# frobelbest/BANet

Hardware: AMD Instinct MI355X
Metric: LM iterations/sec (2-frame 640x480 5-level dense BA, 128-coeff depth basis, batch 32) (higher is better)
Workload: dtype f32 (SYRK: fp32 operands as bf16x3 / scaled fp16x2 pieces, fp32 accumulate, <= 2e-7 per entry; roofline.syrk_form)

## Files before the change

### banet_amd/_capi.py

```python
import ctypes
import os

import torch

_HERE = os.path.dirname(os.path.abspath(__file__))
LIB_PATH = os.environ.get("BANET_HIP_LIB") or os.path.join(_HERE, "lib", "libbanet_hip.so")

LEGACY_LM, LEGACY_FIXED, BUNDLE_CAMERA, BUNDLE = 0, 1, 2, 3

_FP = ctypes.c_void_p


class BanetError(RuntimeError):
    pass


class Level(ctypes.Structure):
    _fields_ = [("B", ctypes.c_int32), ("N", ctypes.c_int32), ("C", ctypes.c_int32), ("K", ctypes.c_int32),
                ("H", ctypes.c_int32), ("W", ctypes.c_int32), ("variant", ctypes.c_int32),
                ("dense", ctypes.c_int32), ("tgt_has_grad", ctypes.c_int32), ("normalize_rays", ctypes.c_int32),
                ("scale", ctypes.c_float), ("pairs", ctypes.c_int32), ("flags", ctypes.c_int32), ("policy", ctypes.c_int32),
                ("src", _FP), ("tgt", _FP), ("depth", _FP), ("basis", _FP), ("rays", _FP),
                ("fx", _FP), ("fy", _FP), ("ox", _FP), ("oy", _FP), ("intr", _FP)]

# ... 42 lines not shown
class Mlp(ctypes.Structure):
    _fields_ = [("w", _FP * 5), ("b", _FP * 5)]


class State(ctypes.Structure):
    _fields_ = [("R", _FP), ("T", _FP), ("Wc", _FP), ("iters", _FP), ("ratio", _FP), ("lambda_out", _FP),
                ("delta", _FP)]


class LmParams(ctypes.Structure):
    _fields_ = [("angle_change", ctypes.c_float), ("translation_change", ctypes.c_float),
                ("residual_ratio", ctypes.c_float), ("solver", ctypes.c_int32)]


SOLVER_QR, SOLVER_INVERSE = 0, 1

EXPORTS = {
    "banet_version": (ctypes.c_int, []),
    "banet_error_string": (ctypes.c_char_p, [ctypes.c_int]),
    "banet_equation_construction_workspace_bytes": (ctypes.c_size_t, [ctypes.c_int] * 4),
    "banet_equation_construction_f32": (ctypes.c_int, [_FP] * 5 + [ctypes.c_int] * 4 + [_FP, ctypes.c_size_t, _FP]),
    "banet_equation_construction_grad_workspace_bytes": (ctypes.c_size_t, [ctypes.c_int] * 4),
    "banet_equation_construction_grad_f32": (ctypes.c_int, [_FP] * 8 + [ctypes.c_int] * 4 + [_FP, ctypes.c_size_t, _FP]),
    "banet_resample_f32": (ctypes.c_int, [_FP] * 3 + [ctypes.c_int] * 6 + [_FP]),
    "banet_target_map_f32": (ctypes.c_int, [_FP] * 2 + [ctypes.c_int] * 4 + [_FP]),
    "banet_depth_output_f32": (ctypes.c_int, [_FP] * 4 + [ctypes.c_int] * 3 + [_FP]),
    "banet_resample_grad_workspace_bytes": (ctypes.c_size_t, [ctypes.c_int] * 6),
    "banet_resample_grad_f32": (ctypes.c_int, [_FP] * 5 + [ctypes.c_int] * 7 + [_FP, ctypes.c_size_t, _FP]),
    "banet_depth_output_grad_workspace_bytes": (ctypes.c_size_t, [ctypes.c_int] * 3),
    "banet_depth_output_grad_f32": (ctypes.c_int, [_FP] * 6 + [ctypes.c_int] * 4 + [_FP, ctypes.c_size_t, _FP]),
# ... 18 lines not shown
    "banet_sample_stats_grad_workspace_bytes": (ctypes.c_size_t, [ctypes.c_int] * 5),
    "banet_sample_stats_grad_det_f32": (ctypes.c_int, [_FP] * 4 + [ctypes.c_int] * 5 + [_FP] * 5 + [_FP, ctypes.c_size_t, _FP]),
    "banet_spd_solve_f32": (ctypes.c_int, [_FP] * 3 + [ctypes.c_int] * 2 + [_FP]),
    "banet_dense_adjoint_workspace_bytes": (ctypes.c_size_t, [ctypes.POINTER(Level)]),
    "banet_dense_adjoint_workspace_bytes_ex": (ctypes.c_size_t, [ctypes.POINTER(Level), ctypes.c_int]),
    "banet_dense_adjoint_f32": (ctypes.c_int, [ctypes.POINTER(Level)] + [_FP] * 11 + [_FP, ctypes.c_size_t, _FP]),
    "banet_dense_adjoint_ex_f32": (ctypes.c_int, [ctypes.POINTER(Level)] + [_FP] * 11 + [ctypes.c_int, _FP, ctypes.c_size_t, _FP]),
    "banet_small_step_adjoint_workspace_bytes": (ctypes.c_size_t, [ctypes.c_int] * 6),
    "banet_small_step_adjoint_f32": (ctypes.c_int, [ctypes.c_int] * 6 + [ctypes.c_float, ctypes.POINTER(Mlp)] + [_FP] * 14 +
                                     [ctypes.POINTER(Mlp), _FP, ctypes.c_size_t, _FP]),
    "banet_target_map_adjoint_f32": (ctypes.c_int, [_FP] * 2 + [ctypes.c_int] * 4 + [_FP]),
    "banet_target_map_adjoint_ex_f32": (ctypes.c_int, [_FP] * 2 + [ctypes.c_int] * 5 + [_FP]),
    "banet_build_id": (ctypes.c_char_p, []),
    "banet_gather_selection": (ctypes.c_int, [_FP]),
    "banet_syrk_selection": (ctypes.c_int, [_FP]),
    "banet_profile_ranges": (ctypes.c_int, [ctypes.c_int]),
    "banet_profile_begin": (ctypes.c_int, [ctypes.c_int]),
    "banet_profile_end": (ctypes.c_int, [ctypes.c_int, ctypes.POINTER(ctypes.c_int32), ctypes.POINTER(ctypes.c_int32),
                                         ctypes.POINTER(ctypes.c_double), ctypes.POINTER(ctypes.c_int32)]),
}

_lib = None


def lib():
    global _lib
    if _lib is None:
        if not os.path.exists(LIB_PATH):
            raise BanetError("%s not found: build it with banet_amd/csrc/build.sh (or __graft_entry__.build())"
                             % LIB_PATH)
# ... 40 lines not shown
```

### banet_amd/csrc/api.hip

```cpp
#include "kernels.hpp"

namespace banet {

static bool aligned256(const void* p) { return (reinterpret_cast<uintptr_t>(p) & 255u) == 0; }

static int check_level(const banet_level_t* lv) {
  if (!lv || !lv->src || !lv->tgt || !lv->depth) return BANET_ERR_INVALID_ARG;
  if (lv->variant < BANET_LEGACY_LM || lv->variant > BANET_BUNDLE) return BANET_ERR_INVALID_ARG;
  if (lv->K > 0 && !lv->basis) return BANET_ERR_INVALID_ARG;
  if ((lv->variant == BANET_BUNDLE) != (lv->K > 0)) return BANET_ERR_INVALID_ARG;
  if (lv->pairs < 0 || (lv->policy != BANET_POLICY_THROUGHPUT && lv->policy != BANET_POLICY_BATCH_INVARIANT)) return BANET_ERR_INVALID_ARG;
  if (lv->pairs > 1 && lv->variant != BANET_BUNDLE && lv->variant != BANET_BUNDLE_CAMERA) return BANET_ERR_INVALID_ARG;
  if (lv->dense) {
    if (!lv->intr || !(lv->scale > 0.f)) return BANET_ERR_INVALID_ARG;
  } else {
    if (!lv->rays || !lv->fx || !lv->fy || !lv->ox || !lv->oy) return BANET_ERR_INVALID_ARG;
  }
  return BANET_OK;
}

struct LevelWs {
  float* partials;
  float* AtA;
  float* Atb;
// ... 34 lines not shown
  a.C = lv->C;
  a.K = lv->K;
  a.pairs = npairs(lv);
  a.P = 6 * a.pairs + lv->K;
  a.variant = lv->variant;
  a.l2_base = l2_base;
  a.max_iters = 0;
  a.use_mlp = lv->variant != BANET_LEGACY_FIXED;
  if (mlp) a.mlp = *mlp;
  else
    for (int i = 0; i < 5; ++i) a.mlp.w[i] = a.mlp.b[i] = nullptr;
  a.AtA = AtA;
  a.Atb = Atb;
  a.absres = absres;
  a.nvalid = nvalid;
  a.st = *st;
  a.ctl = nullptr;
  a.queue = nullptr;
  a.nqueue = 0;
  a.bigA = nullptr;
  a.mlp_y = nullptr;
  a.flags = lv->flags;
  banet_lm_params_default(&a.lm);
  return a;
}

static int check_state(const banet_level_t* lv, const banet_mlp_t* mlp, const banet_state_t* st) {
  if (!st || !st->R || !st->T || !st->iters || !st->ratio || !st->lambda_out || !st->delta) return BANET_ERR_INVALID_ARG;
  if (lv->K > 0 && !st->Wc) return BANET_ERR_INVALID_ARG;
  if (lv->variant != BANET_LEGACY_FIXED) {
// ... 126 lines not shown

size_t banet_lm_level_workspace_bytes(const banet_level_t* lv) {
  AsmPlan pl;
  if (plan_assemble(lv, num_cus(), &pl) != BANET_OK) return 0;
  return carve_level(lv, pl, nullptr).total;
}

void banet_lm_params_default(banet_lm_params_t* p) {
  if (!p) return;
  p->angle_change = (float)(0.002 * (3.14 / 180.0));
  p->translation_change = 0.0002f;
  p->residual_ratio = 1.0f;
  p->solver = BANET_SOLVER_QR;
}

constexpr int kRoleSmallLevel = 19200;

int banet_lm_level_f32(const banet_level_t* lv, const banet_mlp_t* mlp, float l2_base, int max_iters,
                       int early_termination, banet_state_t* st, void* ws, size_t ws_bytes, banet_stream_t stream) {
  return banet_lm_level_ex_f32(lv, mlp, l2_base, max_iters, early_termination, nullptr, st, ws, ws_bytes, stream);
}

int banet_lm_level_ex_f32(const banet_level_t* lv, const banet_mlp_t* mlp, float l2_base, int max_iters,
                          int early_termination, const banet_lm_params_t* params, banet_state_t* st, void* ws,
                          size_t ws_bytes, banet_stream_t stream) {
  int rc = check_level(lv);
  if (rc != BANET_OK) return rc;
  rc = check_state(lv, mlp, st);
  if (rc != BANET_OK) return rc;
  if (max_iters < 0) return BANET_ERR_INVALID_ARG;
  AsmPlan pl;
// ... 20 lines not shown
    for (int it = 0; it <= max_iters; ++it) {
      rc = launch_assemble(lv, pl, st->R, st->T, st->Wc, &w.ctl->active, stride, w.partials, w.AtA, w.Atb, w.absres,
                           w.nvalid, s);
      if (rc != BANET_OK) return rc;
      {
        RangeScope r("solve", lv->N);
        rc = launch_solve(a, s);
      }
      if (rc != BANET_OK) return rc;
    }
  } else {
    launch_zero_iters(st->iters, lv->B, s);
    a.queue = assemble_queue(pl, w.partials);
    a.nqueue = 8 * npairs(lv);
    if (a.queue) launch_zero_iters(a.queue, lv->B * a.nqueue, s);
    const int Bsel = selection_batch(lv);
    const bool role = lv->variant == BANET_BUNDLE && mlp != nullptr && a.use_mlp && syrk_runs_mlp_role(pl.s) && lv->C <= 256 &&
                      (lv->C & 3) == 0 && ((long long)Bsel * (pl.s.Gs + 1) <= num_cus() || (Bsel <= 8 && pl.s.Gs >= 16) ||
                       (lv->N <= kRoleSmallLevel && pl.s.Gs >= 4)) &&
                      !(lv->flags & kDevMlpInSolve);
    if (role) {
      a.mlp_y = w.mlp_y;
      if ((long long)Bsel * (pl.s.Gs + 1) > num_cus()) pl.s.Gs -= 1;
    }
    for (int it = 0; it < max_iters; ++it) {
      rc = launch_assemble(lv, pl, st->R, st->T, st->Wc, nullptr, 0, w.partials, w.AtA, w.Atb, w.absres, w.nvalid, s,
                           a.queue == nullptr, role ? mlp : nullptr, role ? w.mlp_y : nullptr, nullptr,
                           pl.s.f16 ? (it == 0 ? (max_iters > 1 ? 2 : 0) : 1) : -1);
      if (rc != BANET_OK) return rc;
      {
        RangeScope r("solve", lv->N);
        rc = launch_solve(a, s);
      }
      if (rc != BANET_OK) return rc;
    }
  }
  return BANET_OK;
}

int banet_resample_f32(const float* data, const float* warp, float* out, int B, int N, int C, int H, int W, int mode,
                       banet_stream_t stream) {
  if (!data || !warp || !out) return BANET_ERR_INVALID_ARG;
  return launch_resample(data, warp, out, B, N, C, H, W, mode, static_cast<hipStream_t>(stream));
// ... 158 lines not shown
int banet_gather_selection(const banet_level_t* lv) {
  GatherPlan pl;
  const int rc = plan_gather(lv, num_cus(), &pl);
  if (rc != BANET_OK) return rc;
  return pl.quad ? 4 : pl.strip ? 3 : pl.patch ? 2 : pl.c128 ? 1 : 0;
}

int banet_syrk_selection(const banet_level_t* lv) {
  AsmPlan pl;
  const int rc = plan_assemble(lv, num_cus(), &pl);
  if (rc != BANET_OK) return rc;
  if (lv->K == 0) return -1000;
  return pl.s.f16 ? 4 : pl.s.direct;
}

int banet_profile_begin(int max_launches) { return profile_begin(max_launches); }

int banet_profile_end(int max_tags, int32_t* tag_points, int32_t* tag_launches, double* tag_ms, int32_t* ntags) {
  return profile_end(max_tags, tag_points, tag_launches, tag_ms, ntags);
}

}
```

### banet_amd/csrc/assemble.hip

```cpp
#include <atomic>
#include <dlfcn.h>

#include <cstdio>
#include <cstdlib>
#include <vector>

#include "kernels.hpp"

namespace banet {

namespace {
struct Profiler {
  bool on = false;
  std::vector<hipEvent_t> ev;
  std::vector<int> tag;
  int used = 0;
} g_prof;

struct Timed {
  hipStream_t s;
  int slot;
  Timed(hipStream_t st, int tag) : s(st), slot(-1) {
    if (g_prof.on && (size_t)(2 * g_prof.used + 1) < g_prof.ev.size()) {
      slot = g_prof.used++;
// ... 105 lines not shown
      (void)hipGetLastError();
      n = kDefault;
    }
    cached[dev].store(n, std::memory_order_relaxed);
  }
  return n;
}

int* assemble_queue(const AsmPlan& pl, void* ws) {
  return pl.g.c128 ? reinterpret_cast<int*>(static_cast<char*>(ws) + pl.g.off_queue) : nullptr;
}

int launch_assemble(const banet_level_t* lv, const AsmPlan& pl, const float* R, const float* T, const float* Wc,
                    const int32_t* active, int active_stride, void* ws, float* AtA, float* Atb, float* absres,
                    float* nvalid, hipStream_t s, bool reset_queue, const banet_mlp_t* role_mlp, float* role_y,
                    unsigned char* mask_out, int f16_stats) {
  char* base = static_cast<char*>(ws);
  float* gpart = reinterpret_cast<float*>(base);
  float* rec = lv->K > 0 ? reinterpret_cast<float*>(base + pl.off_rec) : nullptr;
  float* spart = lv->K > 0 ? reinterpret_cast<float*>(base + pl.off_spart) : nullptr;
  int rc;
  if (reset_queue) prepare_gather(lv, pl.g, gpart, s);
  {
    RangeScope r("gather", lv->N);
    Timed t(s, lv->N);
    rc = launch_gather(lv, pl.g, R, T, Wc, active, active_stride, rec, gpart, s, mask_out);
  }
  if (rc != BANET_OK) return rc;
  const float* gred;
  {
    RangeScope r("fold", lv->N);
// ... 5 lines not shown
    MlpRole mr{};
    if (role_mlp != nullptr && role_y != nullptr && syrk_runs_mlp_role(pl.s)) {
      mr.gpart = gred;
      mr.grows = pl.g.frows;
      mr.gstride = pl.g.pstride;
      mr.mlp = *role_mlp;
      mr.C = lv->C;
      mr.pairs = npairs(lv);
      mr.Nf = (float)lv->N * (float)npairs(lv);
      mr.y = role_y;
    }
    rc = launch_syrk(lv->basis, rec, lv->B, lv->N, lv->K, npairs(lv), pl.s, active, active_stride, spart, s,
                     mr.y != nullptr ? &mr : nullptr, f16_stats);
    if (rc != BANET_OK) return rc;
  }
  RangeScope r("reduce", lv->N);
  launch_reduce2(gred, pl.g.frows, pl.g.pstride, spart, pl.s.Gs, pl.s.pstride, active, active_stride, lv->B, lv->K, lv->C,
                 npairs(lv), AtA, Atb, absres, nvalid, s);
  return hipGetLastError() == hipSuccess ? BANET_OK : BANET_ERR_LAUNCH;
}

}
```

### banet_amd/csrc/kernels.hpp

```cpp
#pragma once
#include "common.hpp"

namespace banet {

constexpr int kUStrideS = 8;

int num_cus();

void prepare_gather(const banet_level_t* lv, const GatherPlan& pl, float* partials, hipStream_t s);
int launch_gather(const banet_level_t* lv, const GatherPlan& pl, const float* R, const float* T, const float* Wc,
                  const int32_t* active, int active_stride, float* rec, float* partials, hipStream_t s,
                  unsigned char* mask_out = nullptr);
const float* finish_gather(const banet_level_t* lv, const GatherPlan& pl, const int32_t* active, int active_stride,
                           float* partials, hipStream_t s);

struct MlpRole {
  const float* gpart;
  int grows, gstride;
  banet_mlp_t mlp;
  int C, pairs;
  float Nf;
  float* y;
};
int launch_syrk_wide(const float* basis, const float* rec, int B, int N, int K, int pairs, int Gs, int pstride,
                     const int32_t* active, int active_stride, float* partials, float* aux, hipStream_t s,
                     const float* colmax = nullptr, const float* recmax = nullptr);
int launch_syrk(const float* basis, const float* rec, int B, int N, int K, int pairs, const SyrkPlan& pl,
                const int32_t* active, int active_stride, float* partials, hipStream_t s, const MlpRole* mr = nullptr,
                int f16_stats = -1);
inline bool syrk_runs_mlp_role(const SyrkPlan& pl) { return pl.direct == 2; }
void launch_reduce2(const float* gpart, int Gg, int gstride, const float* spart, int Gs, int sstride,
                    const int32_t* active, int active_stride, int B, int K, int C, int pairs, float* AtA, float* Atb,
                    float* absres, float* nvalid, hipStream_t s);

int launch_assemble(const banet_level_t* lv, const AsmPlan& pl, const float* R, const float* T, const float* Wc,
                    const int32_t* active, int active_stride, void* ws, float* AtA, float* Atb, float* absres,
                    float* nvalid, hipStream_t s, bool reset_queue = true, const banet_mlp_t* role_mlp = nullptr,
                    float* role_y = nullptr, unsigned char* mask_out = nullptr, int f16_stats = -1);
int* assemble_queue(const AsmPlan& pl, void* ws);
int profile_ranges(int enable);
struct RangeScope {
  bool on;
  RangeScope(const char* role, int n = -1);
  ~RangeScope();
};
int profile_begin(int max_launches);
int profile_end(int max_tags, int32_t* tag_points, int32_t* tag_launches, double* tag_ms, int32_t* ntags);

int launch_resample(const float* data, const float* warp, float* out, int B, int N, int C, int H, int W, int mode,
                    hipStream_t s);
int launch_target_map(const float* img, float* out, int B, int H, int W, int C, hipStream_t s);
int launch_depth_output(const float* init, const float* basis, const float* Wc, float* out, int B, int N, int K,
                        hipStream_t s);
// ... 34 lines not shown
  float Tprev[3];
  int32_t pad_[3];
};
static_assert(sizeof(LmCtl) == 80, "LmCtl layout");

struct SolveArgs {
  int B, N, C, K, P, variant, pairs;
  float l2_base;
  int max_iters;
  banet_mlp_t mlp;
  int use_mlp;
  const float* AtA;
  const float* Atb;
  const float* absres;
  const float* nvalid;
  banet_state_t st;
  LmCtl* ctl;
  float* bigA;
  int* queue;
  int nqueue;
  const float* mlp_y;
  banet_lm_params_t lm;
  int flags;
};
int launch_solve(const SolveArgs& a, hipStream_t s);
int launch_spd_solve(const float* A, const float* rhs, float* x, int B, int P, hipStream_t s);
bool spd_solve_fits(int P);
size_t solve_big_bytes(int B, int P, int C);
void launch_ctl_init(LmCtl* ctl, int32_t* iters, int B, hipStream_t s);
void launch_zero_iters(int32_t* iters, int B, hipStream_t s);
// ... 27 lines not shown
```

### banet_amd/csrc/plan.hpp

```cpp
#pragma once
#include <stddef.h>
#include <stdint.h>

#include <algorithm>

#include "../../include/banet_hip.h"
#include "dev_flags.hpp"

#ifndef BANET_GATHER_WAVES
#define BANET_GATHER_WAVES 3
#endif
#ifndef BANET_G128P_WAVES
#define BANET_G128P_WAVES 2
#endif
#ifndef BANET_G128_WAVES
#define BANET_G128_WAVES 3
#endif

namespace banet {

constexpr int kWave = 64;
constexpr int kTilePix = 64;
constexpr int kBlock = 256;
constexpr int kNumWaves = kBlock / kWave;
// ... 225 lines not shown
};

inline int plan_assemble(const banet_level_t* lv, int cus, AsmPlan* pl) {
  *pl = AsmPlan{};
  int rc = plan_gather(lv, cus, &pl->g);
  if (rc != BANET_OK) return rc;
  rc = plan_syrk(lv->B, selection_batch(lv), lv->N, lv->K, npairs(lv), lv->flags, cus, &pl->s);
  if (rc != BANET_OK) return rc;
  pl->P = 6 * npairs(lv) + lv->K;
  pl->off_rec = pl->g.partial_bytes;
  pl->off_spart = pl->off_rec + pl->g.rec_bytes;
  pl->ws_bytes = pl->off_spart + pl->s.partial_bytes;
  return BANET_OK;
}

}
```

### banet_amd/csrc/solve.hip

```cpp
#include <type_traits>

#include "kernels.hpp"
#include "mlp.hpp"

namespace banet {

#ifdef BANET_TIMING
__device__ __forceinline__ unsigned long long stick() {
  unsigned long long t;
  asm volatile("s_memtime %0\n\ts_waitcnt lgkmcnt(0)" : "=s"(t)::"memory");
  return t;
}
#define STICK(v) const unsigned long long v = stick()
#else
#define STICK(v)
#endif

constexpr int kSolveThreads = 1024;
[[maybe_unused]] constexpr int kSolveWaves = kSolveThreads / 64;
constexpr int kGrid = 32;

__device__ __forceinline__ float block_sum(float v, float* sred) { return block_sum_t<kSolveThreads>(v, sred); }

__device__ __forceinline__ float wave_sum_fast(float v) {
// ... 569 lines not shown
      float d[2] = {owner ? a12 * x0 : 0.f, owner ? a12 * x1 : 0.f};
      block_sum_n<2>(d, srB);
      const float s = A[(size_t)(n - 1) * ld + n - 1] - d[1];
      const float t = A[(size_t)n * ld + n - 1] - d[0];
      const float xl = t / s;
      if (owner) x[row] = x0 - x1 * xl;
      if (tid == 0) x[n - 1] = xl;
    } else if (owner) {
      x[row] = x0;
    }
  }
  __syncthreads();
  return ok;
}

template <bool BIG>
__global__ __launch_bounds__(kSolveThreads) void ba_solve_update_kernel(const SolveArgs a) {
  extern __shared__ __attribute__((aligned(16))) float smem[];
  const int b = blockIdx.x, tid = threadIdx.x;
  const int P = a.P, C = a.C, K = a.K;
  const bool blocked = P >= kGrid;
  const int ld = blocked ? ldlt_ld(P) : P + 2;
  const int arows = blocked ? P + 4 : P;
  constexpr bool big = BIG;
  float* gA = big ? a.bigA + (size_t)b * solve_big_floats(P) : nullptr;
  float* sA = smem;
  float* sX = sA + (big ? 0 : ((arows * ld + 3) & ~3));
  float* sH0 = sX + ((P + 3) & ~3);
  float* sH1 = sH0 + 4 * C;
  float* sAvg = sH1 + 4 * C;
  float* sRed = sAvg + ((C + 3) & ~3);
  float* sScal = sRed + 20;
  float* sPart = sRed + 24;
  int* sPerm = reinterpret_cast<int*>(sPart + solve_scratch_floats(P));

  LmCtl* ctl = a.ctl ? a.ctl + b : nullptr;
  if (ctl && ctl->active == 0) return;

  STICK(tk0);
  const bool legacy = a.variant == BANET_LEGACY_LM || a.variant == BANET_LEGACY_FIXED;
  const int pairs = a.pairs;
  const float Nf = (float)a.N * (float)pairs;
  const float nval = a.nvalid[b];
  const float numvalid = Nf / nval;
  float ss = 0.f, sm = 0.f;
  for (int c = tid; c < C; c += kSolveThreads) {
    float v = a.absres[(size_t)b * C + c] / Nf;
    if (a.variant == BANET_LEGACY_LM) v = numvalid * v;
    sAvg[c] = v;
    ss += v * v;
    sm += v;
  }
  const float nrm = sqrtf(block_sum(ss, sRed));
  const float avg_scalar = block_sum(sm, sRed) / (float)C;
  float lam;
  if (a.use_mlp && a.mlp_y != nullptr) {
    const float e = legacy ? 1.f : 2.f;
    lam = powf(nrm, e + a.mlp_y[b]);
  } else if (a.use_mlp) {
    __syncthreads();
    mlp_layer(sAvg, sH0, a.mlp.w[0], a.mlp.b[0], C, 2 * C, 0, sPart, sRed);
    mlp_layer(sH0, sH1, a.mlp.w[1], a.mlp.b[1], 2 * C, 4 * C, 0, sPart, sRed);
// ... 17 lines not shown
          for (int i = 0; i < 3; ++i) a.st.T[b * 3 + i] = ctl->Tprev[i];
          ctl->uw = 0.f;
          ctl->ut = 0.f;
        }
        ctl->pending = 0;
      }
      if (!(a.st.iters[b] < a.max_iters && a.lm.angle_change < ctl->uw && a.lm.translation_change < ctl->ut)) {
        ctl->active = 0;
        go = 0;
      }
      sScal[2] = (float)go;
    }
    __syncthreads();
    if (sScal[2] == 0.f) return;
  }
  const float* A_g = a.AtA + (size_t)b * P * P;
  if (big) {
    for (int e = tid; e < P * P; e += kSolveThreads) {
      const int i = e / P, j = e - i * P;
      float v = A_g[e];
      if (i == j && !(a.variant == BANET_BUNDLE && i == P - 1)) v = v + (v + 1e-5f) * lam;
      gA[i * ld + j] = v;
    }
    for (int i = tid; i < P; i += kSolveThreads) gA[P * ld + i] = a.Atb[(size_t)b * P + i];
    __threadfence_block();
  } else {
    for (int e = tid; e < P * P; e += kSolveThreads) {
      const int i = e / P, j = e - i * P;
      float v = A_g[e];
      if (i == j && !(a.variant == BANET_BUNDLE && i == P - 1)) v = v + (v + 1e-5f) * lam;
      sA[i * ld + j] = v;
    }
    for (int i = tid; i < P; i += kSolveThreads) sA[blocked ? P * ld + i : i * ld + P] = a.Atb[(size_t)b * P + i];
  }
  __syncthreads();
  STICK(tk2);
  if (legacy && P == 6) {
    if (tid == 0) {
      float rhs[6];
      for (int i = 0; i < 6; ++i) rhs[i] = sA[i * ld + P];
      if (a.lm.solver == BANET_SOLVER_INVERSE)
        inverse_solve_small(sA, ld, rhs, sX);
      else
        qr_solve_small(sA, ld, rhs, 6, sX);
    }
    __syncthreads();
  } else {
    float* sCol = sPart;
// ... 81 lines not shown
  const size_t fl = (size_t)(big ? 0 : ((arows * ld + 3) & ~3)) + ((P + 3) & ~3) + 8 * C + ((C + 3) & ~3) + 24 +
                    solve_scratch_floats(P) + P + 8;
  return fl * sizeof(float);
}

size_t solve_big_bytes(int B, int P, int C) {
  if (solve_lds_bytes(P, C, false) <= 160 * 1024) return 0;
  return (size_t)B * solve_big_floats(P) * sizeof(float);
}

int launch_solve(const SolveArgs& a, hipStream_t s) {
  const bool need_big = solve_lds_bytes(a.P, a.C, false) > 160 * 1024;
  if (need_big && a.bigA == nullptr) return BANET_ERR_UNSUPPORTED;
  const size_t lds = solve_lds_bytes(a.P, a.C, need_big);
  if (lds > 160 * 1024) return BANET_ERR_UNSUPPORTED;
  if (need_big) {
    if (lds > 64 * 1024)
      (void)hipFuncSetAttribute((const void*)ba_solve_update_kernel<true>, hipFuncAttributeMaxDynamicSharedMemorySize, (int)lds);
    hipLaunchKernelGGL(ba_solve_update_kernel<true>, dim3(a.B), dim3(kSolveThreads), lds, s, a);
  } else {
    if (lds > 64 * 1024)
      (void)hipFuncSetAttribute((const void*)ba_solve_update_kernel<false>, hipFuncAttributeMaxDynamicSharedMemorySize, (int)lds);
    hipLaunchKernelGGL(ba_solve_update_kernel<false>, dim3(a.B), dim3(kSolveThreads), lds, s, a);
  }
  return hipGetLastError() == hipSuccess ? BANET_OK : BANET_ERR_LAUNCH;
}

__global__ __launch_bounds__(kSolveThreads) void spd_solve_kernel(const float* __restrict__ A, const float* __restrict__ rhs,
                                                                  float* __restrict__ x, int P) {
  extern __shared__ __attribute__((aligned(16))) float smem[];
  const int b = blockIdx.x, tid = threadIdx.x;
  const int ld = ldlt_ld(P);
  float* sA = smem;
  float* sX = sA + (((P + 4) * ld + 3) & ~3);
  float* sScr = sX + ((P + 8 + 3) & ~3);
  const float* A_g = A + (size_t)b * P * P;
  for (int e = tid; e < P * P; e += kSolveThreads) {
    const int i = e / P, j = e - i * P;
    sA[i * ld + j] = A_g[e];
// ... 34 lines not shown
```

### banet_amd/csrc/syrk.hip

```cpp
#include <algorithm>
#include "kernels.hpp"
#include "mlp.hpp"
#include "syrk_split.hpp"

namespace banet {

struct SyrkArgs {
  const float* basis;
  const float* rec;
  const int32_t* active;
  int active_stride;
  float* partials;
  int N, K, Gs, tiles, pstride;
  int pairs;
  int pass;
  MlpRole mr;
  const float* colmax;
  const float* recmax;
};

template <int NB>
__global__ __launch_bounds__(kBlock, NB > 8 ? 1 : 2) void ba_syrk_kernel(const SyrkArgs a) {
  constexpr int PW = NB > 8 ? 2 : 1;
  constexpr int KPAD = NB * 16;
// ... 691 lines not shown
          pd[cc * K + rr] = v;
        }
        ++idx;
      }
  }
}

__global__ __launch_bounds__(256) void ba_reduce2_kernel(const float* __restrict__ gpart, int Gg, int gstride,
                                                         const float* __restrict__ spart, int Gs, int sstride,
                                                         const int32_t* active, int active_stride, int K, int C, int pairs,
                                                         float* __restrict__ AtA, float* __restrict__ Atb,
                                                         float* __restrict__ absres, float* __restrict__ nvalid) {
  __shared__ float sQ[4][64];
  const int b = blockIdx.y;
  if (active != nullptr && active[(size_t)b * active_stride] == 0) return;
  const int P6 = 6 * pairs, P = P6 + K;
  const int rq = threadIdx.x >> 6, ej = threadIdx.x & 63;
  const int e = blockIdx.x * 64 + ej;
  const int total = P * P + P + C + 1;
  const bool live = e < total;
  int off = 0, pair = -1;
  bool zero = false;
  float sign = 1.f;
  if (e < P * P) {
    const int i = e / P, j = e - i * P;
    if (i < P6 && j < P6) {
      if (i / 6 != j / 6) {
        zero = true;
      } else {
        pair = i / 6;
        const int ii = i % 6, jj = j % 6;
        const int lo = ii < jj ? ii : jj, hi = ii < jj ? jj : ii;
        off = 6 * lo - lo * (lo - 1) / 2 + (hi - lo);
      }
    } else if (i < P6 || j < P6) {
      const int c = i < P6 ? i : j, k = (i < P6 ? j : i) - P6;
      off = c * K + k;
      sign = -1.f;
    } else {
      off = (P6 + 1) * K + (i - P6) * K + (j - P6);
    }
  } else if (e < P * P + P) {
    const int i = e - P * P;
    if (i < P6) {
      pair = i / 6;
      off = 21 + i % 6;
    } else {
      off = P6 * K + (i - P6);
      sign = -1.f;
    }
  } else if (e < P * P + P + C) {
    pair = -2;
    off = kGHdr + (e - P * P - P);
  } else {
    pair = -2;
    off = 27;
  }
  float v = 0.f;
  const bool from_s = pair == -1;
  if (live && !zero && (from_s || rq == 0)) {
    const int p0 = pair == -2 ? 0 : pair, p1 = pair == -2 ? pairs : pair + 1;
    for (int pp = p0; pp < (from_s ? p0 + 1 : p1); ++pp) {
      const float* p = from_s ? spart + (size_t)b * Gs * sstride + off : gpart + ((size_t)b * pairs + pp) * Gg * gstride + off;
      const size_t st = from_s ? sstride : gstride;
      int i = 0, n = Gg;
      if (from_s) {
        i = (Gs * rq) >> 2;
        n = (Gs * (rq + 1)) >> 2;
      }
      float s0 = 0.f, s1 = 0.f, s2 = 0.f, s3 = 0.f;
      for (; i + 3 < n; i += 4) {
        s0 += p[(size_t)(i + 0) * st];
        s1 += p[(size_t)(i + 1) * st];
        s2 += p[(size_t)(i + 2) * st];
        s3 += p[(size_t)(i + 3) * st];
      }
      for (; i < n; ++i) s0 += p[(size_t)i * st];
      v += (s0 + s1) + (s2 + s3);
    }
    v *= sign;
  }
  sQ[rq][ej] = v;
  __syncthreads();
  if (rq != 0 || !live) return;
  if (from_s && !zero) v = (sQ[0][ej] + sQ[1][ej]) + (sQ[2][ej] + sQ[3][ej]);
  if (e < P * P)
    AtA[(size_t)b * P * P + e] = v;
  else if (e < P * P + P)
    Atb[(size_t)b * P + (e - P * P)] = v;
  else if (e < P * P + P + C)
    absres[(size_t)b * C + (e - P * P - P)] = v;
  else
    nvalid[b] = v;
}

__global__ __launch_bounds__(256) void ba_colmax_kernel(const float* __restrict__ basis, int N, int K, const int32_t* active,
                                                        int active_stride, unsigned* __restrict__ colmax) {
  __shared__ unsigned sMax[256][4];
  const int b = blockIdx.y, tid = threadIdx.x;
  if (active != nullptr && active[(size_t)b * active_stride] == 0) return;
// ... 188 lines not shown
```

### banet_amd/ops.py

```python
import ctypes
from typing import Tuple

import torch

from . import _capi as capi

_VARIANT_OF = {"legacy_lm": capi.LEGACY_LM, "legacy_fixed": capi.LEGACY_FIXED,
               "bundle_camera": capi.BUNDLE_CAMERA, "bundle": capi.BUNDLE}


def _eq_shapes(jacobian, gradient, difference):
    B, N, two, P = jacobian.shape
    Bg, Ng, C, two2 = gradient.shape
    if two != 2 or two2 != 2 or (Bg, Ng) != (B, N) or tuple(difference.shape) != (B, N, C, 1):
        raise capi.BanetError("equation_construction: expected J[B,N,2,P], G[B,N,C,2], d[B,N,C,1]; got %s %s %s"
                              % (tuple(jacobian.shape), tuple(gradient.shape), tuple(difference.shape)))
    return B, N, C, P


def equation_construction_forward(jacobian, gradient, difference):
    J, G, d = capi.f32c(jacobian), capi.f32c(gradient), capi.f32c(difference)
    B, N, C, P = _eq_shapes(J, G, d)
    L = capi.lib()
    left = torch.empty((B, P, P), dtype=torch.float32, device=J.device)
# ... 199 lines not shown
SYRK_THREE_PRODUCTS = capi.DEV_SYRK_THREE_PRODUCTS


SYRK_F16, NO_SYRK_F16 = capi.DEV_SYRK_F16, capi.DEV_NO_SYRK_F16
SYRK_KERNELS = {0: "ba_syrk_kernel", 1: "ba_syrk_direct_kernel", 2: "ba_syrk_bf16x6_kernel (bf16 x 3 pieces, 6 products)",
                3: "syrk_wide.hip jobs", 4: "ba_syrk_bf16x6_kernel (fp16 x 2 pieces, 3 products, scaled)", -1000: "none (K = 0)"}


def syrk_selection(level):
    rc = capi.lib().banet_syrk_selection(ctypes.byref(level.c))
    if rc < 0 and rc != -1000:
        capi.check(rc)
    return rc


def gather_selection(level):
    rc = capi.lib().banet_gather_selection(ctypes.byref(level.c))
    if rc < 0:
        capi.check(rc)
    return rc


def ba_assemble(level, R, T, Wc=None, return_mask=False):
    L = capi.lib()
    dev = level.device
    B, P, C = level.B, level.P, level.C
    AtA = torch.empty((B, P, P), dtype=torch.float32, device=dev)
    Atb = torch.empty((B, P), dtype=torch.float32, device=dev)
    absres = torch.empty((B, C), dtype=torch.float32, device=dev)
    nvalid = torch.empty((B,), dtype=torch.float32, device=dev)
# ... 166 lines not shown
```

### include/banet_hip.h

```cpp
#ifndef BANET_HIP_H_
#define BANET_HIP_H_

#include <stddef.h>
#include <stdint.h>

#ifdef __cplusplus
extern "C" {
#endif

#ifndef BANET_STREAM_T
#define BANET_STREAM_T
typedef void* banet_stream_t;
#endif

#define BANET_VERSION 150

enum {
  BANET_OK = 0,
  BANET_ERR_INVALID_ARG = -1,
  BANET_ERR_WORKSPACE = -2,
  BANET_ERR_UNSUPPORTED = -3,
  BANET_ERR_LAUNCH = -4
};

// ... 163 lines not shown
                                    banet_stream_t stream);

size_t banet_small_step_adjoint_workspace_bytes(int variant, int B, int N, int C, int K, int pairs);
int banet_small_step_adjoint_f32(int variant, int B, int N, int C, int K, int pairs, float l2_regularizer_base,
                                 const banet_mlp_t* mlp, const float* AtA, const float* Atb, const float* absres,
                                 const float* delta, const float* R, const float* T, const float* gR, const float* gT,
                                 const float* gW, float* gAtA, float* gAtb, float* gabs, float* dR, float* dT,
                                 const banet_mlp_t* gmlp, void* ws, size_t ws_bytes, banet_stream_t stream);

int banet_profile_begin(int max_launches);
int banet_profile_end(int max_tags, int32_t* tag_points, int32_t* tag_launches, double* tag_ms,
                      int32_t* ntags);
const char* banet_build_id(void);
int banet_gather_selection(const banet_level_t* lv);
int banet_syrk_selection(const banet_level_t* lv);
int banet_profile_ranges(int enable);

#ifdef __cplusplus
}
#endif
#endif
```

Measured before the change: 24960.

## Fuse partial-sum reduction into the LM solve kernel to drop a launch

The LM loop stops launching the separate reduce2 kernel that folds gather and SYRK partials into AtA/Atb/absres/nvalid. The solve kernel now reads those partials directly, with the symmetric case loading only the upper triangle and mirroring it. This removes one launch per iteration and the write and re-read of AtA. In exchange, each solve block, one per batch item, does the reduction with less parallelism than the dedicated grid had. The fused path is on by default when Gs <= 16 and can be disabled with an environment variable.

```diff
diff --git a/banet_amd/_capi.py b/banet_amd/_capi.py
--- a/banet_amd/_capi.py
+++ b/banet_amd/_capi.py
@@ -80,6 +80,7 @@
 
 
 SOLVER_QR, SOLVER_INVERSE = 0, 1
+LM_TAIL_REDUCE_IN_SOLVE, LM_TAIL_SYRK_HOSTS_MLP = 1 << 20, 1 << 21
 
 EXPORTS = {
     "banet_version": (ctypes.c_int, []),
@@ -128,6 +129,7 @@
     "banet_build_id": (ctypes.c_char_p, []),
     "banet_gather_selection": (ctypes.c_int, [_FP]),
     "banet_syrk_selection": (ctypes.c_int, [_FP]),
+    "banet_lm_tail_selection": (ctypes.c_int, [_FP]),
     "banet_profile_ranges": (ctypes.c_int, [ctypes.c_int]),
     "banet_profile_begin": (ctypes.c_int, [ctypes.c_int]),
     "banet_profile_end": (ctypes.c_int, [ctypes.c_int, ctypes.POINTER(ctypes.c_int32), ctypes.POINTER(ctypes.c_int32),
diff --git a/banet_amd/csrc/api.hip b/banet_amd/csrc/api.hip
--- a/banet_amd/csrc/api.hip
+++ b/banet_amd/csrc/api.hip
@@ -1,3 +1,6 @@
+#include <cstdlib>
+#include <cstring>
+
 #include "kernels.hpp"
 
 namespace banet {
@@ -72,6 +75,8 @@
   a.Atb = Atb;
   a.absres = absres;
   a.nvalid = nvalid;
+  a.gpart = a.spart = nullptr;
+  a.Gg = a.gstride = a.Gs = a.sstride = a.ssym = 0;
   a.st = *st;
   a.ctl = nullptr;
   a.queue = nullptr;
@@ -228,7 +233,10 @@
   p->solver = BANET_SOLVER_QR;
 }
 
-constexpr int kRoleSmallLevel = 19200;
+static bool lm_tail_unfused() {
+  const char* e = std::getenv("BANET_LM_TAIL");
+  return e != nullptr && std::strcmp(e, "unfused") == 0;
+}
 
 int banet_lm_level_f32(const banet_level_t* lv, const banet_mlp_t* mlp, float l2_base, int max_iters,
                        int early_termination, banet_state_t* st, void* ws, size_t ws_bytes, banet_stream_t stream) {
@@ -279,19 +287,24 @@
     a.queue = assemble_queue(pl, w.partials);
     a.nqueue = 8 * npairs(lv);
     if (a.queue) launch_zero_iters(a.queue, lv->B * a.nqueue, s);
-    const int Bsel = selection_batch(lv);
-    const bool role = lv->variant == BANET_BUNDLE && mlp != nullptr && a.use_mlp && syrk_runs_mlp_role(pl.s) && lv->C <= 256 &&
-                      (lv->C & 3) == 0 && ((long long)Bsel * (pl.s.Gs + 1) <= num_cus() || (Bsel <= 8 && pl.s.Gs >= 16) ||
-                       (lv->N <= kRoleSmallLevel && pl.s.Gs >= 4)) &&
-                      !(lv->flags & kDevMlpInSolve);
-    if (role) {
-      a.mlp_y = w.mlp_y;
-      if ((long long)Bsel * (pl.s.Gs + 1) > num_cus()) pl.s.Gs -= 1;
+    const LmTailPlan tail = plan_lm_tail(lv, pl, num_cus(), true, lm_tail_unfused());
+    const bool role = tail.role && mlp != nullptr && a.use_mlp;
+    if (role) a.mlp_y = w.mlp_y;
+    pl.s.Gs = tail.Gs;
+    const bool fused = tail.reduce_in_solve != 0;
+    if (fused) {
+      a.AtA = a.Atb = a.absres = a.nvalid = nullptr;
+      a.Gg = pl.g.frows;
+      a.gstride = pl.g.pstride;
+      a.spart = lv->K > 0 ? reinterpret_cast<const float*>(reinterpret_cast<const char*>(w.partials) + pl.off_spart) : nullptr;
+      a.Gs = lv->K > 0 ? pl.s.Gs : 0;
+      a.sstride = pl.s.pstride;
+      a.ssym = pl.s.direct == 2 ? 1 : 0;
     }
     for (int it = 0; it < max_iters; ++it) {
-      rc = launch_assemble(lv, pl, st->R, st->T, st->Wc, nullptr, 0, w.partials, w.AtA, w.Atb, w.absres, w.nvalid, s,
-                           a.queue == nullptr, role ? mlp : nullptr, role ? w.mlp_y : nullptr, nullptr,
-                           pl.s.f16 ? (it == 0 ? (max_iters > 1 ? 2 : 0) : 1) : -1);
+      rc = launch_assemble(lv, pl, st->R, st->T, st->Wc, nullptr, 0, w.partials, fused ? nullptr : w.AtA, w.Atb, w.absres,
+                           w.nvalid, s, a.queue == nullptr, role ? mlp : nullptr, role ? w.mlp_y : nullptr, nullptr,
+                           pl.s.f16 ? (it == 0 ? (max_iters > 1 ? 2 : 0) : 1) : -1, fused ? &a.gpart : nullptr);
       if (rc != BANET_OK) return rc;
       {
         RangeScope r("solve", lv->N);
@@ -480,6 +493,14 @@
   return pl.s.f16 ? 4 : pl.s.direct;
 }
 
+int banet_lm_tail_selection(const banet_level_t* lv) {
+  AsmPlan pl;
+  const int rc = plan_assemble(lv, num_cus(), &pl);
+  if (rc != BANET_OK) return rc;
+  const LmTailPlan t = plan_lm_tail(lv, pl, num_cus(), true, lm_tail_unfused());
+  return t.launches | (t.Gs << 8) | (t.reduce_in_solve ? BANET_LM_TAIL_REDUCE_IN_SOLVE : 0) | (t.role ? BANET_LM_TAIL_SYRK_HOSTS_MLP : 0);
+}
+
 int banet_profile_begin(int max_launches) { return profile_begin(max_launches); }
 
 int banet_profile_end(int max_tags, int32_t* tag_points, int32_t* tag_launches, double* tag_ms, int32_t* ntags) {
diff --git a/banet_amd/csrc/assemble.hip b/banet_amd/csrc/assemble.hip
--- a/banet_amd/csrc/assemble.hip
+++ b/banet_amd/csrc/assemble.hip
@@ -143,7 +143,7 @@
 int launch_assemble(const banet_level_t* lv, const AsmPlan& pl, const float* R, const float* T, const float* Wc,
                     const int32_t* active, int active_stride, void* ws, float* AtA, float* Atb, float* absres,
                     float* nvalid, hipStream_t s, bool reset_queue, const banet_mlp_t* role_mlp, float* role_y,
-                    unsigned char* mask_out, int f16_stats) {
+                    unsigned char* mask_out, int f16_stats, const float** gred_out) {
   char* base = static_cast<char*>(ws);
   float* gpart = reinterpret_cast<float*>(base);
   float* rec = lv->K > 0 ? reinterpret_cast<float*>(base + pl.off_rec) : nullptr;
@@ -179,6 +179,8 @@
                      mr.y != nullptr ? &mr : nullptr, f16_stats);
     if (rc != BANET_OK) return rc;
   }
+  if (gred_out != nullptr) *gred_out = gred;
+  if (AtA == nullptr) return hipGetLastError() == hipSuccess ? BANET_OK : BANET_ERR_LAUNCH;
   RangeScope r("reduce", lv->N);
   launch_reduce2(gred, pl.g.frows, pl.g.pstride, spart, pl.s.Gs, pl.s.pstride, active, active_stride, lv->B, lv->K, lv->C,
                  npairs(lv), AtA, Atb, absres, nvalid, s);
diff --git a/banet_amd/csrc/kernels.hpp b/banet_amd/csrc/kernels.hpp
--- a/banet_amd/csrc/kernels.hpp
+++ b/banet_amd/csrc/kernels.hpp
@@ -36,7 +36,8 @@
 int launch_assemble(const banet_level_t* lv, const AsmPlan& pl, const float* R, const float* T, const float* Wc,
                     const int32_t* active, int active_stride, void* ws, float* AtA, float* Atb, float* absres,
                     float* nvalid, hipStream_t s, bool reset_queue = true, const banet_mlp_t* role_mlp = nullptr,
-                    float* role_y = nullptr, unsigned char* mask_out = nullptr, int f16_stats = -1);
+                    float* role_y = nullptr, unsigned char* mask_out = nullptr, int f16_stats = -1,
+                    const float** gred_out = nullptr);
 int* assemble_queue(const AsmPlan& pl, void* ws);
 int profile_ranges(int enable);
 struct RangeScope {
@@ -101,6 +102,11 @@
   const float* Atb;
   const float* absres;
   const float* nvalid;
+  const float* gpart;
+  int Gg, gstride;
+  const float* spart;
+  int Gs, sstride;
+  int ssym;
   banet_state_t st;
   LmCtl* ctl;
   float* bigA;
diff --git a/banet_amd/csrc/plan.hpp b/banet_amd/csrc/plan.hpp
--- a/banet_amd/csrc/plan.hpp
+++ b/banet_amd/csrc/plan.hpp
@@ -263,4 +263,30 @@
   return BANET_OK;
 }
 
-}
+constexpr int kRoleSmallLevel = 19200;
+constexpr int kTailSolveMaxGs = 16;
+
+struct LmTailPlan {
+  int role;
+  int Gs;
+  int reduce_in_solve;
+  int launches;
+};
+
+inline LmTailPlan plan_lm_tail(const banet_level_t* lv, const AsmPlan& pl, int cus, bool fixed_count = true, bool unfused = false) {
+  LmTailPlan t{};
+  const int Bsel = selection_batch(lv);
+  t.Gs = pl.s.Gs;
+  t.role = (fixed_count && lv->variant == BANET_BUNDLE && pl.s.direct == 2 && lv->C <= 256 && (lv->C & 3) == 0 &&
+            ((long long)Bsel * (pl.s.Gs + 1) <= cus || (Bsel <= 8 && pl.s.Gs >= 16) || (lv->N <= kRoleSmallLevel && pl.s.Gs >= 4)) &&
+            !(lv->flags & kDevMlpInSolve)) ? 1 : 0;
+  if (t.role && (long long)Bsel * (pl.s.Gs + 1) > cus) t.Gs -= 1;
+  t.reduce_in_solve = (fixed_count && !unfused && t.Gs <= kTailSolveMaxGs) ? 1 : 0;
+  const int pairs = npairs(lv);
+  const int syrk = lv->K == 0 ? 0 : (pl.s.direct ? 1 : pairs);
+  const int recmax = (lv->K > 0 && pl.s.f16 && fixed_count) ? 1 : 0;
+  t.launches = 1 + (pl.g.frows != pl.g.rows ? 1 : 0) + recmax + syrk + (t.reduce_in_solve ? 0 : 1) + 1;
+  return t;
+}
+
+}
diff --git a/banet_amd/csrc/reduce2.hpp b/banet_amd/csrc/reduce2.hpp
--- /dev/null
+++ b/banet_amd/csrc/reduce2.hpp
@@ -0,0 +1,89 @@
+#pragma once
+#include "kernels.hpp"
+
+namespace banet {
+
+struct Reduce2Elem {
+  int off;
+  int pair;
+  bool zero;
+  float sign;
+};
+
+__device__ __forceinline__ Reduce2Elem reduce2_elem(int e, int K, int C, int pairs) {
+  const int P6 = 6 * pairs, P = P6 + K;
+  Reduce2Elem m;
+  m.off = 0;
+  m.pair = -1;
+  m.zero = false;
+  m.sign = 1.f;
+  if (e < P * P) {
+    const int i = e / P, j = e - i * P;
+    if (i < P6 && j < P6) {
+      if (i / 6 != j / 6) {
+        m.zero = true;
+      } else {
+        m.pair = i / 6;
+        const int ii = i % 6, jj = j % 6;
+        const int lo = ii < jj ? ii : jj, hi = ii < jj ? jj : ii;
+        m.off = 6 * lo - lo * (lo - 1) / 2 + (hi - lo);
+      }
+    } else if (i < P6 || j < P6) {
+      const int c = i < P6 ? i : j, k = (i < P6 ? j : i) - P6;
+      m.off = c * K + k;
+      m.sign = -1.f;
+    } else {
+      m.off = (P6 + 1) * K + (i - P6) * K + (j - P6);
+    }
+  } else if (e < P * P + P) {
+    const int i = e - P * P;
+    if (i < P6) {
+      m.pair = i / 6;
+      m.off = 21 + i % 6;
+    } else {
+      m.off = P6 * K + (i - P6);
+      m.sign = -1.f;
+    }
+  } else if (e < P * P + P + C) {
+    m.pair = -2;
+    m.off = kGHdr + (e - P * P - P);
+  } else {
+    m.pair = -2;
+    m.off = 27;
+  }
+  return m;
+}
+
+__device__ __forceinline__ float reduce2_rows(const float* __restrict__ p, size_t st, int i, int n) {
+  float s0 = 0.f, s1 = 0.f, s2 = 0.f, s3 = 0.f;
+  for (; i + 3 < n; i += 4) {
+    s0 += p[(size_t)(i + 0) * st];
+    s1 += p[(size_t)(i + 1) * st];
+    s2 += p[(size_t)(i + 2) * st];
+    s3 += p[(size_t)(i + 3) * st];
+  }
+  for (; i < n; ++i) s0 += p[(size_t)i * st];
+  return (s0 + s1) + (s2 + s3);
+}
+
+__device__ __forceinline__ float reduce2_gather(const float* __restrict__ gpart, int Gg, int gstride, int b, int pairs,
+                                                const Reduce2Elem& m) {
+  const int p0 = m.pair == -2 ? 0 : m.pair, p1 = m.pair == -2 ? pairs : m.pair + 1;
+  float v = 0.f;
+  for (int pp = p0; pp < p1; ++pp)
+    v += reduce2_rows(gpart + ((size_t)b * pairs + pp) * Gg * gstride + m.off, (size_t)gstride, 0, Gg);
+  return v * m.sign;
+}
+
+template <int GS = 0>
+__device__ __forceinline__ float reduce2_syrk_run(const float* __restrict__ spart, int Gs_, int sstride, int b,
+                                                  const Reduce2Elem& m, int rq) {
+  const int Gs = GS > 0 ? GS : Gs_;
+  float v = 0.f;
+  v += reduce2_rows(spart + (size_t)b * Gs * sstride + m.off, (size_t)sstride, (Gs * rq) >> 2, (Gs * (rq + 1)) >> 2);
+  return v * m.sign;
+}
+
+__device__ __forceinline__ float reduce2_syrk_join(float q0, float q1, float q2, float q3) { return (q0 + q1) + (q2 + q3); }
+
+}
diff --git a/banet_amd/csrc/solve.hip b/banet_amd/csrc/solve.hip
--- a/banet_amd/csrc/solve.hip
+++ b/banet_amd/csrc/solve.hip
@@ -2,6 +2,7 @@
 
 #include "kernels.hpp"
 #include "mlp.hpp"
+#include "reduce2.hpp"
 
 namespace banet {
 
@@ -607,7 +608,49 @@
   return ok;
 }
 
-template <bool BIG>
+__device__ __forceinline__ float damp_diag(float v, float lam) { return v + (v + 1e-5f) * lam; }
+
+template <int GS>
+__device__ __forceinline__ float fused_entry(const SolveArgs& a, int b, int e) {
+  const Reduce2Elem m = reduce2_elem(e, a.K, a.C, a.pairs);
+  if (m.zero) return 0.f;
+  if (m.pair != -1) return reduce2_gather(a.gpart, a.Gg, a.gstride, b, a.pairs, m);
+  const float q0 = reduce2_syrk_run<GS>(a.spart, a.Gs, a.sstride, b, m, 0);
+  const float q1 = reduce2_syrk_run<GS>(a.spart, a.Gs, a.sstride, b, m, 1);
+  const float q2 = reduce2_syrk_run<GS>(a.spart, a.Gs, a.sstride, b, m, 2);
+  const float q3 = reduce2_syrk_run<GS>(a.spart, a.Gs, a.sstride, b, m, 3);
+  return reduce2_syrk_join(q0, q1, q2, q3);
+}
+
+template <int GS>
+__device__ __forceinline__ void fused_load(const SolveArgs& a, int b, float* A, int ld, bool blocked, float lam) {
+  const int tid = threadIdx.x, P = a.P;
+  const bool undamped_last = a.variant == BANET_BUNDLE;
+  if (a.ssym) {
+    const int T = P * (P + 1) / 2;
+#pragma unroll 2
+    for (int t = tid; t < T; t += kSolveThreads) {
+      int i = (int)((sqrtf(8.f * (float)t + 1.f) - 1.f) * 0.5f);
+      while ((i + 1) * (i + 2) / 2 <= t) ++i;
+      while (i * (i + 1) / 2 > t) --i;
+      const int j = t - i * (i + 1) / 2;
+      float v = fused_entry<GS>(a, b, i * P + j);
+      if (i == j && !(undamped_last && i == P - 1)) v = damp_diag(v, lam);
+      A[i * ld + j] = v;
+      A[j * ld + i] = v;
+    }
+  } else {
+    for (int e = tid; e < P * P; e += kSolveThreads) {
+      const int i = e / P, j = e - i * P;
+      float v = fused_entry<GS>(a, b, e);
+      if (i == j && !(undamped_last && i == P - 1)) v = damp_diag(v, lam);
+      A[i * ld + j] = v;
+    }
+  }
+  for (int i = tid; i < P; i += kSolveThreads) A[blocked ? P * ld + i : i * ld + P] = fused_entry<GS>(a, b, P * P + i);
+}
+
+template <bool BIG, bool FUSED>
 __global__ __launch_bounds__(kSolveThreads) void ba_solve_update_kernel(const SolveArgs a) {
   extern __shared__ __attribute__((aligned(16))) float smem[];
   const int b = blockIdx.x, tid = threadIdx.x;
@@ -634,11 +677,19 @@
   const bool legacy = a.variant == BANET_LEGACY_LM || a.variant == BANET_LEGACY_FIXED;
   const int pairs = a.pairs;
   const float Nf = (float)a.N * (float)pairs;
-  const float nval = a.nvalid[b];
+  if constexpr (FUSED) {
+    for (int c = tid; c <= C; c += kSolveThreads) {
+      const float v = reduce2_gather(a.gpart, a.Gg, a.gstride, b, pairs, reduce2_elem(P * P + P + c, K, C, pairs));
+      if (c < C) sAvg[c] = v;
+      else sScal[3] = v;
+    }
+    __syncthreads();
+  }
+  const float nval = FUSED ? sScal[3] : a.nvalid[b];
   const float numvalid = Nf / nval;
   float ss = 0.f, sm = 0.f;
   for (int c = tid; c < C; c += kSolveThreads) {
-    float v = a.absres[(size_t)b * C + c] / Nf;
+    float v = (FUSED ? sAvg[c] : a.absres[(size_t)b * C + c]) / Nf;
     if (a.variant == BANET_LEGACY_LM) v = numvalid * v;
     sAvg[c] = v;
     ss += v * v;
@@ -686,12 +737,22 @@
     __syncthreads();
     if (sScal[2] == 0.f) return;
   }
+  if constexpr (FUSED) {
+    float* A = big ? gA : sA;
+    switch (a.Gs) {
+      case 5: fused_load<5>(a, b, A, ld, blocked, lam); break;
+      case 7: fused_load<7>(a, b, A, ld, blocked, lam); break;
+      case 8: fused_load<8>(a, b, A, ld, blocked, lam); break;
+      default: fused_load<0>(a, b, A, ld, blocked, lam); break;
+    }
+    if (big) __threadfence_block();
+  } else {
   const float* A_g = a.AtA + (size_t)b * P * P;
   if (big) {
     for (int e = tid; e < P * P; e += kSolveThreads) {
       const int i = e / P, j = e - i * P;
       float v = A_g[e];
-      if (i == j && !(a.variant == BANET_BUNDLE && i == P - 1)) v = v + (v + 1e-5f) * lam;
+      if (i == j && !(a.variant == BANET_BUNDLE && i == P - 1)) v = damp_diag(v, lam);
       gA[i * ld + j] = v;
     }
     for (int i = tid; i < P; i += kSolveThreads) gA[P * ld + i] = a.Atb[(size_t)b * P + i];
@@ -700,10 +761,11 @@
     for (int e = tid; e < P * P; e += kSolveThreads) {
       const int i = e / P, j = e - i * P;
       float v = A_g[e];
-      if (i == j && !(a.variant == BANET_BUNDLE && i == P - 1)) v = v + (v + 1e-5f) * lam;
+      if (i == j && !(a.variant == BANET_BUNDLE && i == P - 1)) v = damp_diag(v, lam);
       sA[i * ld + j] = v;
     }
     for (int i = tid; i < P; i += kSolveThreads) sA[blocked ? P * ld + i : i * ld + P] = a.Atb[(size_t)b * P + i];
+  }
   }
   __syncthreads();
   STICK(tk2);
@@ -815,15 +877,12 @@
   if (need_big && a.bigA == nullptr) return BANET_ERR_UNSUPPORTED;
   const size_t lds = solve_lds_bytes(a.P, a.C, need_big);
   if (lds > 160 * 1024) return BANET_ERR_UNSUPPORTED;
-  if (need_big) {
-    if (lds > 64 * 1024)
-      (void)hipFuncSetAttribute((const void*)ba_solve_update_kernel<true>, hipFuncAttributeMaxDynamicSharedMemorySize, (int)lds);
-    hipLaunchKernelGGL(ba_solve_update_kernel<true>, dim3(a.B), dim3(kSolveThreads), lds, s, a);
-  } else {
-    if (lds > 64 * 1024)
-      (void)hipFuncSetAttribute((const void*)ba_solve_update_kernel<false>, hipFuncAttributeMaxDynamicSharedMemorySize, (int)lds);
-    hipLaunchKernelGGL(ba_solve_update_kernel<false>, dim3(a.B), dim3(kSolveThreads), lds, s, a);
-  }
+  const bool fused = a.gpart != nullptr;
+  if (fused && a.ctl != nullptr) return BANET_ERR_INVALID_ARG;
+  auto k = need_big ? (fused ? ba_solve_update_kernel<true, true> : ba_solve_update_kernel<true, false>)
+                    : (fused ? ba_solve_update_kernel<false, true> : ba_solve_update_kernel<false, false>);
+  if (lds > 64 * 1024) (void)hipFuncSetAttribute((const void*)k, hipFuncAttributeMaxDynamicSharedMemorySize, (int)lds);
+  hipLaunchKernelGGL(k, dim3(a.B), dim3(kSolveThreads), lds, s, a);
   return hipGetLastError() == hipSuccess ? BANET_OK : BANET_ERR_LAUNCH;
 }
 
diff --git a/banet_amd/csrc/syrk.hip b/banet_amd/csrc/syrk.hip
--- a/banet_amd/csrc/syrk.hip
+++ b/banet_amd/csrc/syrk.hip
@@ -1,6 +1,7 @@
 #include <algorithm>
 #include "kernels.hpp"
 #include "mlp.hpp"
+#include "reduce2.hpp"
 #include "syrk_split.hpp"
 
 namespace banet {
@@ -729,76 +730,22 @@
   __shared__ float sQ[4][64];
   const int b = blockIdx.y;
   if (active != nullptr && active[(size_t)b * active_stride] == 0) return;
-  const int P6 = 6 * pairs, P = P6 + K;
+  const int P = 6 * pairs + K;
   const int rq = threadIdx.x >> 6, ej = threadIdx.x & 63;
   const int e = blockIdx.x * 64 + ej;
   const int total = P * P + P + C + 1;
   const bool live = e < total;
-  int off = 0, pair = -1;
-  bool zero = false;
-  float sign = 1.f;
-  if (e < P * P) {
-    const int i = e / P, j = e - i * P;
-    if (i < P6 && j < P6) {
-      if (i / 6 != j / 6) {
-        zero = true;
-      } else {
-        pair = i / 6;
-        const int ii = i % 6, jj = j % 6;
-        const int lo = ii < jj ? ii : jj, hi = ii < jj ? jj : ii;
-        off = 6 * lo - lo * (lo - 1) / 2 + (hi - lo);
-      }
-    } else if (i < P6 || j < P6) {
-      const int c = i < P6 ? i : j, k = (i < P6 ? j : i) - P6;
-      off = c * K + k;
-      sign = -1.f;
-    } else {
-      off = (P6 + 1) * K + (i - P6) * K + (j - P6);
-    }
-  } else if (e < P * P + P) {
-    const int i = e - P * P;
-    if (i < P6) {
-      pair = i / 6;
-      off = 21 + i % 6;
-    } else {
-      off = P6 * K + (i - P6);
-      sign = -1.f;
-    }
-  } else if (e < P * P + P + C) {
-    pair = -2;
-    off = kGHdr + (e - P * P - P);
-  } else {
-    pair = -2;
-    off = 27;
-  }
+  const Reduce2Elem m = reduce2_elem(e, K, C, pairs);
+  const bool zero = m.zero, from_s = m.pair == -1;
   float v = 0.f;
-  const bool from_s = pair == -1;
-  if (live && !zero && (from_s || rq == 0)) {
-    const int p0 = pair == -2 ? 0 : pair, p1 = pair == -2 ? pairs : pair + 1;
-    for (int pp = p0; pp < (from_s ? p0 + 1 : p1); ++pp) {
-      const float* p = from_s ? spart + (size_t)b * Gs * sstride + off : gpart + ((size_t)b * pairs + pp) * Gg * gstride + off;
-      const size_t st = from_s ? sstride : gstride;
-      int i = 0, n = Gg;
-      if (from_s) {
-        i = (Gs * rq) >> 2;
-        n = (Gs * (rq + 1)) >> 2;
-      }
-      float s0 = 0.f, s1 = 0.f, s2 = 0.f, s3 = 0.f;
-      for (; i + 3 < n; i += 4) {
-        s0 += p[(size_t)(i + 0) * st];
-        s1 += p[(size_t)(i + 1) * st];
-        s2 += p[(size_t)(i + 2) * st];
-        s3 += p[(size_t)(i + 3) * st];
-      }
-      for (; i < n; ++i) s0 += p[(size_t)i * st];
-      v += (s0 + s1) + (s2 + s3);
-    }
-    v *= sign;
+  if (live && !zero) {
+    if (from_s) v = reduce2_syrk_run(spart, Gs, sstride, b, m, rq);
+    else if (rq == 0) v = reduce2_gather(gpart, Gg, gstride, b, pairs, m);
   }
   sQ[rq][ej] = v;
   __syncthreads();
   if (rq != 0 || !live) return;
-  if (from_s && !zero) v = (sQ[0][ej] + sQ[1][ej]) + (sQ[2][ej] + sQ[3][ej]);
+  if (from_s && !zero) v = reduce2_syrk_join(sQ[0][ej], sQ[1][ej], sQ[2][ej], sQ[3][ej]);
   if (e < P * P)
     AtA[(size_t)b * P * P + e] = v;
   else if (e < P * P + P)
diff --git a/banet_amd/ops.py b/banet_amd/ops.py
--- a/banet_amd/ops.py
+++ b/banet_amd/ops.py
@@ -237,6 +237,14 @@
     return rc
 
 
+def lm_tail_selection(level):
+    rc = capi.lib().banet_lm_tail_selection(ctypes.byref(level.c))
+    if rc < 0:
+        capi.check(rc)
+    return {"launches": rc & 255, "Gs": (rc >> 8) & 4095, "reduce_in_solve": bool(rc & capi.LM_TAIL_REDUCE_IN_SOLVE),
+            "syrk_hosts_mlp": bool(rc & capi.LM_TAIL_SYRK_HOSTS_MLP)}
+
+
 def gather_selection(level):
     rc = capi.lib().banet_gather_selection(ctypes.byref(level.c))
     if rc < 0:
diff --git a/include/banet_hip.h b/include/banet_hip.h
--- a/include/banet_hip.h
+++ b/include/banet_hip.h
@@ -201,6 +201,8 @@
 const char* banet_build_id(void);
 int banet_gather_selection(const banet_level_t* lv);
 int banet_syrk_selection(const banet_level_t* lv);
+enum { BANET_LM_TAIL_REDUCE_IN_SOLVE = 1 << 20, BANET_LM_TAIL_SYRK_HOSTS_MLP = 1 << 21 };
+int banet_lm_tail_selection(const banet_level_t* lv);
 int banet_profile_ranges(int enable);
 
 #ifdef __cplusplus
```

Result: no change. 24840 (-0.5%).
